# chanchanchan97/ICAFusion

Measured on NVIDIA H100. Metric: 640x512 RGB+IR pairs/sec end-to-end, higher is better.
Workload: dtype f16

## Files before the change

icafusion_b200/csrc/conv_common.cuh:

```cuda
#pragma once
#include "icaf_internal.cuh"

namespace icaf {

constexpr int BM = 128;
constexpr int BK = 64;
constexpr int kLag = 2;
constexpr int kThreads = 288;

enum AMode { A_GATHER = 0, A_TMA2D = 1, A_TMA4D = 2 };

struct ConvProblem {
  const __half* x; const float* bias; const __half* res; __half* y;
  const float* alpha; const float* beta;
  long long x_ld, res_ld, y_ld;
  const float2* ln_stats;
  const float* ln_s;
  float2* stats_out;
};
struct ConvParams {
  ConvProblem p[2];
  int M, N, K, k_pad;
  int B, Hi, Wi, Cin, Ho, Wo, kh, kw, stride, pad;
  int act, epi;
// ... 128 lines not shown
          const float2 r2 = __half22float2(rh[e]);
          rf[2 * e] = r2.x; rf[2 * e + 1] = r2.y;
        }
      } else {
#pragma unroll
        for (int e = 0; e < 8; ++e) rf[e] = 0.f;
      }
      float v[8];
#pragma unroll
      for (int e = 0; e < 8; ++e) v[e] = f(q * 8 + e, rf[e]);
      uint4 o;
      o.x = pack_half2(v[0], v[1]); o.y = pack_half2(v[2], v[3]);
      o.z = pack_half2(v[4], v[5]); o.w = pack_half2(v[6], v[7]);
      if (XM == 2) {
        const __half2* oh = reinterpret_cast<const __half2*>(&o);
#pragma unroll
        for (int e = 0; e < 4; ++e) {
          const float2 w = __half22float2(oh[e]);
          ex.sum += w.x + w.y;
          ex.sumsq += w.x * w.x + w.y * w.y;
        }
      }
      if (do_store) *reinterpret_cast<uint4*>(yp + q * 8) = o;
    }
  } else {
#pragma unroll
    for (int j = 0; j < 32; ++j) {
      if (j < ncols) {
        const float t = f(j, RES != 0 ? __half2float(rp[j]) : 0.f);
        const __half h = __float2half_rn(t);
        if (XM == 2) { const float w = __half2float(h); ex.sum += w; ex.sumsq += w * w; }
        yp[j] = h;
      }
    }
  }
}

__device__ __forceinline__ void load_staged(uint32_t (&acc)[32], const float* p) {
#pragma unroll
  for (int q = 0; q < 8; ++q) {
    const float4 v = *reinterpret_cast<const float4*>(p + 4 * q);
    acc[4 * q] = __float_as_uint(v.x); acc[4 * q + 1] = __float_as_uint(v.y);
    acc[4 * q + 2] = __float_as_uint(v.z); acc[4 * q + 3] = __float_as_uint(v.w);
  }
}

template <bool XM>
__device__ __forceinline__ void epi_dispatch(int mode_act, const uint32_t (&acc)[32], const float* sb, float rbias, float alpha,
                                             float beta, const __half* rp, __half* yp, bool vec, int ncols, EpiRow& ex, int cb) {
  if (XM) {
    switch (mode_act) {
      case 9: epi_chunk<0, 0, 1>(acc, sb, rbias, alpha, beta, rp, yp, vec, ncols, ex, cb); break;
      case 10: epi_chunk<2, 0, 1>(acc, sb, rbias, alpha, beta, rp, yp, vec, ncols, ex, cb); break;
      default: epi_chunk<0, 2, 2>(acc, sb, rbias, alpha, beta, rp, yp, vec, ncols, ex, cb); break;
    }
  } else {
    switch (mode_act) {
      case 0: epi_chunk<0, 0>(acc, sb, rbias, alpha, beta, rp, yp, vec, ncols, ex, cb); break;
      case 1: epi_chunk<0, 1>(acc, sb, rbias, alpha, beta, rp, yp, vec, ncols, ex, cb); break;
      case 2: epi_chunk<0, 2>(acc, sb, rbias, alpha, beta, rp, yp, vec, ncols, ex, cb); break;
      case 3: epi_chunk<1, 0>(acc, sb, rbias, alpha, beta, rp, yp, vec, ncols, ex, cb); break;
      case 4: epi_chunk<1, 1>(acc, sb, rbias, alpha, beta, rp, yp, vec, ncols, ex, cb); break;
      case 5: epi_chunk<1, 2>(acc, sb, rbias, alpha, beta, rp, yp, vec, ncols, ex, cb); break;
      case 6: epi_chunk<2, 0>(acc, sb, rbias, alpha, beta, rp, yp, vec, ncols, ex, cb); break;
      case 7: epi_chunk<2, 1>(acc, sb, rbias, alpha, beta, rp, yp, vec, ncols, ex, cb); break;
      default: epi_chunk<2, 2>(acc, sb, rbias, alpha, beta, rp, yp, vec, ncols, ex, cb); break;
    }
  }
}

template <bool XM>
__device__ __forceinline__ int epi_mode_act(const ConvParams& P, bool has_res) {
  if (XM) return P.ln_parts > 0 ? (P.act == ICAF_ACT_GELU ? 10 : 9) : 11;
  return P.act * 3 + ((P.epi & ICAF_EPI_SCALED_RES) ? 2 : (has_res ? 1 : 0));
}

template <bool XM>
__device__ __forceinline__ void epi_staged_chunk(int mode_act, const uint32_t (&acc)[32], StagedRow& r, const float* sbias,
                                                 float alpha, float beta, int cb, int nb, int N) {
  const int ncols = min(32, N - nb);
  const bool vec = ncols == 32 && ((reinterpret_cast<uintptr_t>(r.yrow + nb) & 15) == 0) &&
                   (!r.rrow || (reinterpret_cast<uintptr_t>(r.rrow + nb) & 15) == 0);
  epi_dispatch<XM>(mode_act, acc, sbias + cb, r.rbias, alpha, beta, r.rrow ? r.rrow + nb : nullptr, r.yrow + nb, vec, ncols,
                   r.ex, cb);
}

constexpr int kOutHalfBytes = BM * 64 * 2;

template <int PP, int NA>
__device__ __forceinline__ void take_cols16(const float (&acc0)[NA], const float (&acc1)[NA], float (&v)[16]) {
  constexpr int Q = PP < NA / 8 ? PP : NA / 8 - 1;
#pragma unroll
  for (int e = 0; e < 8; ++e) { v[e] = acc0[8 * Q + e]; v[8 + e] = acc1[8 * Q + e]; }
}

template <int ACT, int RES>
__device__ __forceinline__ void epi_fragments(const float (&v)[16], uint32_t sa, const float* sb, const float (&rb)[4],
                                              float alpha, float beta) {
#pragma unroll
  for (int h = 0; h < 2; ++h) {
    uint32_t r[4];
    if (RES != 0) ldmatrix_x4(r, sa + 8192u * h);
#pragma unroll
    for (int k = 0; k < 4; ++k) {
      const float2 b = *reinterpret_cast<const float2*>(sb + 8 * (k >> 1));
      const float rbias = rb[2 * h + (k & 1)];
      float2 rf = make_float2(0.f, 0.f);
      if (RES != 0) rf = __half22float2(*reinterpret_cast<const __half2*>(&r[k]));
      r[k] = pack_half2(epi_value<ACT, RES>(v[8 * h + 2 * k], b.x, rbias, rf.x, alpha, beta),
                        epi_value<ACT, RES>(v[8 * h + 2 * k + 1], b.y, rbias, rf.y, alpha, beta));
    }
    stmatrix_x4(sa + 8192u * h, r);
  }
}

__device__ __forceinline__ void epi_fragments_dispatch(int mode_act, const float (&v)[16], uint32_t sa, const float* sb,
                                                       const float (&rb)[4], float alpha, float beta) {
  switch (mode_act) {
    case 0: epi_fragments<0, 0>(v, sa, sb, rb, alpha, beta); break;
    case 1: epi_fragments<0, 1>(v, sa, sb, rb, alpha, beta); break;
    case 2: epi_fragments<0, 2>(v, sa, sb, rb, alpha, beta); break;
    case 3: epi_fragments<1, 0>(v, sa, sb, rb, alpha, beta); break;
    case 4: epi_fragments<1, 1>(v, sa, sb, rb, alpha, beta); break;
    case 5: epi_fragments<1, 2>(v, sa, sb, rb, alpha, beta); break;
    case 6: epi_fragments<2, 0>(v, sa, sb, rb, alpha, beta); break;
    case 7: epi_fragments<2, 1>(v, sa, sb, rb, alpha, beta); break;
    default: epi_fragments<2, 2>(v, sa, sb, rb, alpha, beta); break;
  }
}

template <int NA>
__device__ __forceinline__ void epi_tile_fragments(int mode_act, const float (&acc0)[NA], const float (&acc1)[NA], uint32_t sout,
                                                   const float* sbias, const float (&rb)[4], float alpha, float beta, int w, int l) {
  const uint32_t sa = sout + uint32_t(16 * w + (l & 7) + 8 * ((l >> 3) & 1)) * 128u;
  const float* sb = sbias + 2 * (l & 3);
#pragma unroll 1
  for (int p = 0; p < NA / 8; ++p) {
    float v[16];
    switch (p) {
      case 0: take_cols16<0>(acc0, acc1, v); break;
      case 1: take_cols16<1>(acc0, acc1, v); break;
      case 2: take_cols16<2>(acc0, acc1, v); break;
      case 3: take_cols16<3>(acc0, acc1, v); break;
      case 4: take_cols16<4>(acc0, acc1, v); break;
      case 5: take_cols16<5>(acc0, acc1, v); break;
      case 6: take_cols16<6>(acc0, acc1, v); break;
      default: take_cols16<7>(acc0, acc1, v); break;
    }
    const uint32_t a = sa + uint32_t(p >> 2) * uint32_t(kOutHalfBytes) + (uint32_t((2 * (p & 3) + (l >> 4)) ^ (l & 7)) << 4);
    epi_fragments_dispatch(mode_act, v, a, sb + 16 * p, rb, alpha, beta);
  }
}

__device__ __forceinline__ void fragment_row_bias(float (&rb)[4], const ConvParams& P, const ConvProblem& pr, const TileOrigin& o,
                                                  int w, int l) {
  if ((P.epi & ICAF_EPI_BIAS_ROW) && pr.bias) {
#pragma unroll
    for (int q = 0; q < 4; ++q) {
      int mq;
      bool vq;
      tile_row(P, o, 16 * w + (l >> 2) + 8 * (q & 1) + 64 * (q >> 1), mq, vq);
      rb[q] = vq ? __ldg(pr.bias + mq) : 0.f;
    }
  }
}

template <int BN>
__device__ __forceinline__ void tma_store_tile(const ConvParams& P, const CUtensorMap* map, uint32_t s, int n0, const TileOrigin& o) {
  const int halves = (BN == 128 && n0 + 64 < P.N) ? 2 : 1;
  for (int hh = 0; hh < halves; ++hh) {
    const uint32_t src = s + uint32_t(hh * kOutHalfBytes);
    if (P.a_mode == A_TMA4D) tma_store_4d(map, src, n0 + 64 * hh, o.ox0, o.oy0, o.tb);
    else tma_store_2d(map, src, n0 + 64 * hh, o.m0);
  }
  bulk_commit_group();
}

template <int BN>
__device__ __forceinline__ void tma_load_tile(const ConvParams& P, const CUtensorMap* map, uint32_t s, uint32_t bar, int n0,
                                              const TileOrigin& o) {
  const int halves = (BN == 128 && n0 + 64 < P.N) ? 2 : 1;
  const uint32_t half_bytes = P.a_mode == A_TMA4D ? uint32_t(P.tw * P.th) * 128u : uint32_t(kOutHalfBytes);
  mbar_arrive_expect_tx(bar, uint32_t(halves) * half_bytes);
  for (int hh = 0; hh < halves; ++hh) {
    const uint32_t dst = s + uint32_t(hh * kOutHalfBytes);
    if (P.a_mode == A_TMA4D) tma_load_4d(dst, map, bar, n0 + 64 * hh, o.ox0, o.oy0, o.tb);
    else tma_load_2d(dst, map, bar, n0 + 64 * hh, o.m0);
  }
}

struct ConvPlan {
  int kernel;
  int bn;
  unsigned grid_x, grid_y, grid_z, cluster;
  int smem;
  int tiles, m_tiles, n_tiles;
  int sms;
  bool persist;
  bool stem;
  bool xm;
  int ctas;
};

}
```

icafusion_b200/csrc/conv_gemm.cu:

```cuda
#include <cstdlib>
#include <cstring>

#include "conv_common.cuh"

namespace icaf {

constexpr int kMaxStages = 10;
template <int BN>
struct SmemLayout {
  static constexpr int kABytes = BM * BK * 2;
  static constexpr int kBBytes = BN * BK * 2;
  static constexpr int kStageBytes = kABytes + kBBytes;
  static constexpr int kPitch = BN + 4;
  static constexpr int kAccBytes = BM * kPitch * 4;
  static constexpr int kTailBytes = 256 + BN * 4 + 1024;
  __host__ __device__ static int region(int stages) { return stages * kStageBytes > kAccBytes ? stages * kStageBytes : kAccBytes; }
  static int total(int stages) { return region(stages) + kTailBytes; }
};


template <int BN, bool kTmaA>
__device__ __forceinline__ void load_stage(const ConvParams& P, int a_mode, uint32_t sa, uint32_t bar, uint32_t bytes,
                                           const CUtensorMap* mw, const CUtensorMap* ma, int kb, int n0, const TileOrigin& o) {
  mbar_arrive_expect_tx(bar, bytes);
// ... 379 lines not shown
    mbar_init(order_bar(1), 4);
    mbar_init(res_bar(0), 1);
    mbar_init(res_bar(1), 1);
    for (int h = 0; h < kHaloSlots; ++h) {
      mbar_init(halo_full(h), 1);
      mbar_init(halo_empty(h), 4);
    }
    fence_mbar_init();
  }
  if (tid == 32) {
    tma_prefetch_desc(&maps.w[0]);
    tma_prefetch_desc(&maps.a[0]);
    if (P.tiles > P.m_tiles * P.n_tiles) { tma_prefetch_desc(&maps.w[1]); tma_prefetch_desc(&maps.a[1]); }
    if (!XM) {
      tma_prefetch_desc(&maps.y[0]);
      if (has_res) tma_prefetch_desc(&maps.res[0]);
    }
  }
  __syncthreads();
  pdl_wait();

  if (wg == 0) {
    setmaxnreg_dec<40>();
    if (tid < 32 && elect_one()) {
      const uint32_t a_bytes = a_mode == A_TMA2D ? L::kABytes : uint32_t(P.tw * P.th) * 128u;
      const uint32_t bytes = L::kBBytes + a_bytes;
      int s = 0, h = 0;
      uint32_t ph = 0, hph = 0;
      for (int tile = blockIdx.x; tile < P.tiles; tile += gridDim.x) {
        const PersistTile pt = persist_tile(P, tile);
        const CUtensorMap* mw = pt.z ? &maps.w[1] : &maps.w[0];
        const CUtensorMap* ma = pt.z ? &maps.a[1] : &maps.a[0];
        if (halo) {
          const uint32_t halo_tx = uint32_t((P.tw + 2) * (P.th + 2)) * 128u;
          for (int cb = 0; cb < ncb; ++cb) {
            mbar_wait_quiet(halo_empty(h), hph ^ 1);
            mbar_arrive_expect_tx(halo_full(h), halo_tx);
            tma_load_4d(smem_base + uint32_t(kStages * PL::kFilterBytes + h * P.halo_bytes), ma, halo_full(h), cb * BK,
                        pt.o.ox0 - 1, pt.o.oy0 - 1, pt.o.tb);
            if (++h == kHaloSlots) { h = 0; hph ^= 1; }
            for (int tap = 0; tap < 9; ++tap) {
              mbar_wait_quiet(empty_bar(s), ph ^ 1);
              mbar_arrive_expect_tx(full_bar(s), PL::kFilterBytes);
              tma_load_2d(smem_base + uint32_t(s * PL::kFilterBytes), mw, full_bar(s), tap * P.Cin + cb * BK, pt.n0);
              if (++s == kStages) { s = 0; ph ^= 1; }
            }
          }
          continue;
        }
        for (int kb = 0; kb < nkb; ++kb) {
          mbar_wait_quiet(empty_bar(s), ph ^ 1);
          load_stage<128, true>(P, a_mode, smem_base + s * L::kStageBytes, full_bar(s), bytes, mw, ma, kb, pt.n0, pt.o);
          if (++s == kStages) { s = 0; ph ^= 1; }
        }
      }
    }
    return;
  }

  setmaxnreg_inc<232>();
  const int c = wg - 1;
  const int t = tid & 127, w = t >> 5, l = t & 31;
  const int bar_id = 2 + c;
  const uint32_t sout = smem_base + ring_bytes + uint32_t(c * PL::kOutBytes);
  float* sacc = reinterpret_cast<float*>(smem_gen + ring_bytes + c * PL::kOutBytes);
  float* sbias = reinterpret_cast<float*>(smem_gen + bar_off + 256 + c * 128 * 4);
  int lane_px[2];
#pragma unroll
  for (int hm = 0; hm < 2; ++hm) {
    int m = 64 * hm + 16 * w + (l & 7) + 8 * ((l >> 3) & 1);
    if (m > P.tw * P.th - 1) m = P.tw * P.th - 1;
    const int py = P.tw ? m / P.tw : 0;
    lane_px[hm] = py * (P.tw + 2) + m - py * P.tw;
  }
  for (int tile = blockIdx.x + c * gridDim.x; tile < P.tiles; tile += 2 * gridDim.x) {
    const int j = (tile - int(blockIdx.x)) / int(gridDim.x);
    const PersistTile pt = persist_tile(P, tile);
    const ConvProblem pr = pick_problem(P, pt.z);
    const int n0 = pt.n0;
    const TileOrigin& o = pt.o;
    const float bias_r = (pr.bias && !(P.epi & ICAF_EPI_BIAS_ROW) && n0 + t < P.N) ? __ldg(pr.bias + n0 + t) : 0.f;
    float alpha = 0.f, beta = 1.f;
    if (P.epi & ICAF_EPI_SCALED_RES) { alpha = __ldg(pr.alpha); beta = __ldg(pr.beta); }
    StagedRow sr;
    float rb[4] = {0.f, 0.f, 0.f, 0.f};
    if (XM) {
      staged_row<128, XM>(sr, P, pr, o, t, n0);
    } else {
      fragment_row_bias(rb, P, pr, o, w, l);
      if (t == 0) {
        bulk_wait_group_read<0>();
        if (has_res) tma_load_tile<128>(P, pt.z ? &maps.res[1] : &maps.res[0], sout, res_bar(c), n0, o);
      }
      sbias[t] = bias_r;
      named_bar_sync(bar_id, 128);
    }

    float acc0[64], acc1[64];
#pragma unroll
    for (int i = 0; i < 64; ++i) { acc0[i] = 0.f; acc1[i] = 0.f; }
    auto hand_back = [&](int s) { if (l == 0) mbar_arrive(empty_bar(s)); };
    auto halo_back = [&](int h) { if (l == 0) mbar_arrive(halo_empty(h)); };
    const int g0 = j * nkb;
    if (j > 0) mbar_wait_quiet(order_bar(c), uint32_t((j >> 1) - (1 - c)) & 1u);
    int s_last, h_last = 0;
    if (halo) {
      halo_mma_loop(acc0, acc1, P, smem_base, kStages, g0, j * ncb, lane_px, l, full_bar, halo_full, hand_back, halo_back,
                    s_last, h_last);
    } else {
      s_last = mma_loop<128>(acc0, acc1, smem_base, kStages, nkb, g0 % kStages, uint32_t(g0 / kStages) & 1u, full_bar,
                             hand_back);
    }
    if (l == 0) mbar_arrive(order_bar(c ^ 1));
    wgmma_wait<0>();
    hand_back(s_last);
    if (halo) halo_back(h_last);

    if constexpr (!XM) {
      if (has_res) mbar_wait_quiet(res_bar(c), uint32_t(j >> 1) & 1u);
      epi_tile_fragments<64>(epi_mode_act<false>(P, has_res), acc0, acc1, sout, sbias, rb, alpha, beta, w, l);
      fence_proxy_async_smem();
      named_bar_sync(bar_id, 128);
      if (t == 0) {
        tma_store_tile<128>(P, pt.z ? &maps.y[1] : &maps.y[0], sout, n0, o);
        if (tile + 2 * int(gridDim.x) >= P.tiles) bulk_wait_group<0>();
      }
      continue;
    }

    const int mode_act = epi_mode_act<XM>(P, has_res);
    const float* arow = sacc + size_t(t) * PL::kPitch;
#pragma unroll 1
    for (int cc = 0; cc < 4; ++cc) {
      named_bar_sync(bar_id, 128);
      if (cc == 0) sbias[t] = bias_r;
      switch (cc) {
        case 0: stage_chunk<0>(acc0, acc1, sacc, w, l); break;
        case 1: stage_chunk<1>(acc0, acc1, sacc, w, l); break;
        case 2: stage_chunk<2>(acc0, acc1, sacc, w, l); break;
        default: stage_chunk<3>(acc0, acc1, sacc, w, l); break;
      }
      named_bar_sync(bar_id, 128);
      const int cb = 32 * cc;
      if (sr.mvalid && n0 + cb < P.N) {
        uint32_t acc[32];
        load_staged(acc, arow);
        epi_staged_chunk<XM>(mode_act, acc, sr, sbias, alpha, beta, cb, n0 + cb, P.N);
      }
    }
    if (mode_act == 11 && sr.mvalid && n0 < P.N) epi_row_emit(sr.ex, P, pr, sr.m, n0, min(n0 + 128, P.N));
  }
}

constexpr int kStemThreads = 128;
struct StemLayout {
  static constexpr int kFilterBytes = 3 * SmemLayout<64>::kBBytes;
  static constexpr int kBiasOff = kFilterBytes;
  static constexpr int kBarOff = kBiasOff + 64 * 4;
  static constexpr int kHaloOff = kFilterBytes + 1024;
  __host__ __device__ static int pitch(int Wo) { return (Wo < BM ? Wo : BM) + 2; }
  __host__ __device__ static int runs(int Wo) { return 1 + (BM - 1 + Wo - 1) / Wo; }
  static int total(int Wo) {
    const int halo = runs(Wo) * 3 * pitch(Wo) * 32;
    return kHaloOff + (halo > kOutHalfBytes ? halo : kOutHalfBytes) + 1024;
  }
};

__global__ void __launch_bounds__(kStemThreads, 4)
conv_stem_kernel(const ConvParams P, const __grid_constant__ ConvMaps maps) {
  extern __shared__ uint8_t smem_raw[];
  using SL = StemLayout;
  const uint32_t smem_base = (smem_u32(smem_raw) + 1023u) & ~1023u;
  uint8_t* smem_gen = smem_raw + (smem_base - smem_u32(smem_raw));
  const uint32_t bar = smem_base + SL::kBarOff;
  const uint32_t halo = smem_base + SL::kHaloOff;
  float* sbias = reinterpret_cast<float*>(smem_gen + SL::kBiasOff);

  pdl_launch_dependents();
  const int t = threadIdx.x, w = t >> 5, l = t & 31;
  const int bz = blockIdx.z, n0 = blockIdx.y * 64;
  const ConvProblem pr = pick_problem(P, bz);
  const TileOrigin o{int(blockIdx.x) * BM, 0, 0, 0};
  const int g0 = o.m0 / P.Wo, ox0 = o.m0 - g0 * P.Wo;
  const int len0 = min(P.Wo - ox0, BM);
  const int nruns = 1 + (BM - len0 + P.Wo - 1) / P.Wo;
  const int pitch = SL::pitch(P.Wo);
  int lane_hp[2];
#pragma unroll
  for (int hm = 0; hm < 2; ++hm) {
    const int r = 64 * hm + 16 * w + (l & 7) + 8 * ((l >> 3) & 1);
    int j = 0, p = r;
    if (r >= len0) {
      const int q = (r - len0) / P.Wo;
      j = 1 + q;
      p = r - len0 - q * P.Wo;
    }
    lane_hp[hm] = 3 * j * pitch + p;
  }
  if (t == 0) {
    mbar_init(bar, 1);
    fence_mbar_init();
  }
  if (t == 32) {
    tma_prefetch_desc(bz ? &maps.w[1] : &maps.w[0]);
    tma_prefetch_desc(bz ? &maps.y[1] : &maps.y[0]);
  }
  __syncthreads();
  pdl_wait();

  if (t == 0) {
    const CUtensorMap* mw = bz ? &maps.w[1] : &maps.w[0];
    mbar_arrive_expect_tx(bar, SL::kFilterBytes);
#pragma unroll 1
    for (int kb = 0; kb < 3; ++kb) tma_load_2d(smem_base + uint32_t(kb * SmemLayout<64>::kBBytes), mw, bar, kb * BK, n0);
  }
  if (t < 64) sbias[t] = (pr.bias && !(P.epi & ICAF_EPI_BIAS_ROW) && n0 + t < P.N) ? __ldg(pr.bias + n0 + t) : 0.f;
  float rb[4] = {0.f, 0.f, 0.f, 0.f};
  fragment_row_bias(rb, P, pr, o, w, l);

  const int c = t & 1;
#pragma unroll 1
  for (int j = 0; j < nruns; ++j) {
    const int g = g0 + j;
    const int xs = j ? 0 : ox0;
    const int len = j ? min(P.Wo, BM - len0 - (j - 1) * P.Wo) : len0;
    const int b = g / P.Ho, oy = g - b * P.Ho;
    const bool gv = g < P.B * P.Ho;
#pragma unroll
    for (int ty = 0; ty < 3; ++ty) {
      const int iy = oy + ty - 1;
      const bool rv = gv && (unsigned)iy < (unsigned)P.Hi;
      const __half* src = pr.x + (rv ? (size_t(b) * P.Hi + iy) * P.Wi * pr.x_ld : 0) + 8 * c;
      const int h0 = (3 * j + ty) * pitch;
      for (int px = t >> 1; px < len + 2; px += kStemThreads / 2) {
        const int ix = xs - 1 + px, h = h0 + px;
        const bool ok = rv && (unsigned)ix < (unsigned)P.Wi;
        cp_async16(halo + uint32_t(h) * 32u + (uint32_t(c ^ ((h >> 2) & 1)) << 4), ok ? src + size_t(ix) * pr.x_ld : pr.x, ok);
      }
    }
  }
  cp_async_commit();
  cp_async_wait<0>();
  __syncthreads();
  mbar_wait_quiet(bar, 0);

  float acc0[32], acc1[32];
#pragma unroll
  for (int i = 0; i < 32; ++i) { acc0[i] = 0.f; acc1[i] = 0.f; }
  uint32_t fa[3][2][4];
#pragma unroll
  for (int tap = 0; tap < 9; ++tap) {
    const int f = tap % 3;
    const int off = (tap / 3) * pitch + tap % 3;
#pragma unroll
    for (int hm = 0; hm < 2; ++hm) {
      const int h = lane_hp[hm] + off;
      ldmatrix_x4(fa[f][hm], halo + uint32_t(h) * 32u + (uint32_t((l >> 4) ^ ((h >> 2) & 1)) << 4));
    }
    wgmma_fence();
    const uint64_t bd = gmma_desc_sw128(smem_base + uint32_t((tap >> 2) * SmemLayout<64>::kBBytes + 32 * (tap & 3)));
    wgmma_rs<0>(acc0, fa[f][0], bd, tap != 0);
    wgmma_rs<0>(acc1, fa[f][1], bd, tap != 0);
    wgmma_commit();
    wgmma_wait<2>();
  }
  wgmma_wait<0>();
  __syncthreads();

  epi_tile_fragments<32>(epi_mode_act<false>(P, false), acc0, acc1, halo, sbias, rb, 0.f, 1.f, w, l);
  fence_proxy_async_smem();
  __syncthreads();
  if (t == 0) {
    tma_store_tile<64>(P, bz ? &maps.y[1] : &maps.y[0], halo, n0, o);
    bulk_wait_group<0>();
  }
}

struct SimtParams { ConvParams P; const __half* w[2]; };
__global__ void conv_gemm_simt_kernel(const SimtParams S) {
  pdl_launch_dependents();
  pdl_wait();
  const ConvParams& P = S.P;
  const ConvProblem pr = pick_problem(P, blockIdx.z);
  const __half* w = blockIdx.z ? S.w[1] : S.w[0];
  long long idx = blockIdx.x * (long long)blockDim.x + threadIdx.x;
  if (idx >= (long long)P.M * P.N) return;
  int n = int(idx % P.N);
  int m = int(idx / P.N);
  int ox = m % P.Wo, t = m / P.Wo, oy = t % P.Ho, b = t / P.Ho;
  float acc = 0.f;
  for (int ky = 0; ky < P.kh; ++ky)
    for (int kx = 0; kx < P.kw; ++kx) {
      int iy = oy * P.stride - P.pad + ky, ix = ox * P.stride - P.pad + kx;
      if ((unsigned)iy >= (unsigned)P.Hi || (unsigned)ix >= (unsigned)P.Wi) continue;
      const __half* xp = pr.x + (size_t(b) * P.Hi * P.Wi + size_t(iy) * P.Wi + ix) * pr.x_ld;
      const __half* wp = w + size_t(n) * P.k_pad + (ky * P.kw + kx) * P.Cin;
      for (int c = 0; c < P.Cin; ++c) acc += __half2float(xp[c]) * __half2float(wp[c]);
    }
  if (pr.bias) acc += (P.epi & ICAF_EPI_BIAS_ROW) ? pr.bias[m] : pr.bias[n];
  if (P.act == ICAF_ACT_SILU) acc = acc / (1.0f + expf(-acc));
  else if (P.act == ICAF_ACT_GELU) acc = gelu_erf_f(acc);
  if (pr.res) {
    float rf = __half2float(pr.res[size_t(m) * pr.res_ld + n]);
    acc = (P.epi & ICAF_EPI_SCALED_RES) ? (*pr.alpha) * rf + (*pr.beta) * acc : acc + rf;
  }
  pr.y[size_t(m) * pr.y_ld + n] = __float2half_rn(acc);
}

static int fill_geom(const icaf_conv_geom* g, int n_io, ConvParams& P) {
  if (!g || n_io < 1 || n_io > 2) return set_error(ICAF_ERR_BAD_ARG, "conv2d: need 1 or 2 problems");
  if (!(g->Cin == 4 || g->Cin % 8 == 0)) return set_error(ICAF_ERR_UNSUPPORTED, "conv2d: Cin must be 4 or a multiple of 8");
  if (g->Cin == 4 && (g->Wi % 2 || g->stride % 2 || g->pad % 2 || g->kw % 2))
    return set_error(ICAF_ERR_UNSUPPORTED, "conv2d: packed-image (Cin=4) path needs even Wi, stride, pad, kw");
  if (g->k_pad % 64 || g->k_pad < g->kh * g->kw * g->Cin) return set_error(ICAF_ERR_BAD_ARG, "conv2d: bad k_pad");
  if (g->w_rows < g->Cout) return set_error(ICAF_ERR_BAD_ARG, "conv2d: w_rows < Cout");
  long long M = (long long)g->B * g->Ho * g->Wo;
  if (M <= 0 || M > 0x7fffffffLL || (long long)g->B * g->Hi * g->Wi > 0x7fffffffLL)
    return set_error(ICAF_ERR_BAD_ARG, "conv2d: size out of range");
  if ((g->epi & (ICAF_EPI_ADD_RES | ICAF_EPI_SCALED_RES)) == (ICAF_EPI_ADD_RES | ICAF_EPI_SCALED_RES))
    return set_error(ICAF_ERR_BAD_ARG, "conv2d: ADD_RES and SCALED_RES are exclusive");
  if ((g->epi & ICAF_EPI_LN_FOLD) && ((g->epi & ~ICAF_EPI_LN_FOLD) != 0 || !(g->act == ICAF_ACT_NONE || g->act == ICAF_ACT_GELU) ||
                                      g->kh != 1 || g->kw != 1 || g->stride != 1 || g->pad != 0))
    return set_error(ICAF_ERR_UNSUPPORTED, "conv2d: LN_FOLD is a linear-layer (1x1) epilogue without residual, activation none / GELU");
  if ((g->epi & ICAF_EPI_EMIT_STATS) && ((g->epi & ~ICAF_EPI_EMIT_STATS) != ICAF_EPI_SCALED_RES || g->act != ICAF_ACT_NONE))
    return set_error(ICAF_ERR_UNSUPPORTED, "conv2d: EMIT_STATS rides on the SCALED_RES epilogue without activation");
  P.M = int(M); P.N = g->Cout; P.K = g->kh * g->kw * g->Cin; P.k_pad = g->k_pad;
  P.B = g->B; P.Hi = g->Hi; P.Wi = g->Wi; P.Cin = g->Cin; P.Ho = g->Ho; P.Wo = g->Wo;
  P.kh = g->kh; P.kw = g->kw; P.stride = g->stride; P.pad = g->pad; P.act = g->act; P.epi = g->epi;
  P.a_mode = A_GATHER; P.tw = P.th = P.tiles_x = P.tiles_y = 0; P.stages = 2; P.splits = 1; P.cblk = 64;
  P.ln_parts = 0; P.ln_eps = 0.f; P.ln_inv_k = 0.f;
  P.m_tiles = P.n_tiles = P.tiles = 0;
  P.tma_epi = 0;
  P.halo_bytes = 0;
  memset(P.p, 0, sizeof(P.p));
  return ICAF_OK;
}

static int fill_params(const icaf_conv_geom* g, const icaf_conv_io* io, int n_io, ConvParams& P, const __half* (&w)[2]) {
  if (!io) return set_error(ICAF_ERR_BAD_ARG, "conv2d: null io");
  if (int rc = fill_geom(g, n_io, P)) return rc;
  for (int i = 0; i < 2; ++i) {
    const icaf_conv_io& s = io[i < n_io ? i : 0];
    bool need_res = g->epi & (ICAF_EPI_ADD_RES | ICAF_EPI_SCALED_RES);
    if (!s.x || !s.w || !s.y || (need_res && !s.res) || ((g->epi & ICAF_EPI_SCALED_RES) && (!s.alpha || !s.beta)))
      return set_error(ICAF_ERR_BAD_ARG, "conv2d: null pointer");
    if ((reinterpret_cast<uintptr_t>(s.x) & 15) || (reinterpret_cast<uintptr_t>(s.w) & 15) || (s.x_ld % 8 && g->Cin != 4) ||
        (g->Cin == 4 && s.x_ld != 4))
      return set_error(ICAF_ERR_BAD_ARG, "conv2d: x / w must be 16-byte aligned with x_ld a multiple of 8");
    if ((g->epi & ICAF_EPI_LN_FOLD) && (!s.ln_stats || !s.ln_colsum || s.ln_parts < 1 || s.ln_parts > 64))
      return set_error(ICAF_ERR_BAD_ARG, "conv2d: LN_FOLD needs ln_stats, ln_colsum and 1..64 partials per row");
    if ((g->epi & ICAF_EPI_EMIT_STATS) && !s.stats_out) return set_error(ICAF_ERR_BAD_ARG, "conv2d: EMIT_STATS needs stats_out");
    if (i > 0 && (g->epi & ICAF_EPI_LN_FOLD) && (s.ln_parts != io[0].ln_parts || s.ln_eps != io[0].ln_eps))
      return set_error(ICAF_ERR_BAD_ARG, "conv2d: grouped problems must share ln_parts / ln_eps");
    P.p[i] = ConvProblem{(const __half*)s.x, s.bias, need_res ? (const __half*)s.res : nullptr, (__half*)s.y, s.alpha, s.beta,
                         s.x_ld, s.res_ld, s.y_ld,
                         (g->epi & ICAF_EPI_LN_FOLD) ? (const float2*)s.ln_stats : nullptr,
                         (g->epi & ICAF_EPI_LN_FOLD) ? s.ln_colsum : nullptr,
                         (g->epi & ICAF_EPI_EMIT_STATS) ? (float2*)s.stats_out : nullptr};
    if (i == 0 && (g->epi & ICAF_EPI_LN_FOLD)) { P.ln_parts = s.ln_parts; P.ln_eps = s.ln_eps; P.ln_inv_k = 1.0f / float(P.K); }
    w[i] = (const __half*)s.w;
  }
  return ICAF_OK;
}

static void plan_a_mode(const icaf_conv_geom* g, ConvParams& P) {
  if (g->kh == 1 && g->kw == 1 && g->stride == 1 && g->pad == 0 && g->Cin % 8 == 0) {
    P.a_mode = A_TMA2D;
    return;
  }
  if (g->Cin % 64 == 0 && g->stride <= 2) {
    int best_tw = 0, best_th = 0;
    double best_u = 0.0;
    for (int tw = 1; tw <= 128 && tw <= g->Wo; ++tw) {
      if (g->Wo % tw || tw * g->stride > 256) continue;
      int th = 128 / tw;
      if (th > g->Ho) th = g->Ho;
      if (th * g->stride > 256) th = 256 / g->stride;
      int ty = (g->Ho + th - 1) / th;
      double u = double(g->Wo) * g->Ho / (double(g->Wo / tw) * ty * 128.0);
      if (u > best_u + 1e-9 || (u > best_u - 1e-9 && tw > best_tw)) { best_u = u; best_tw = tw; best_th = th; }
    }
    if (best_u >= 0.6) {
      P.a_mode = A_TMA4D; P.tw = best_tw; P.th = best_th; P.tiles_x = g->Wo / best_tw; P.tiles_y = (g->Ho + best_th - 1) / best_th;
    }
  }
}

template <int BN>
static int plan_tc(ConvParams& P, int n_io, ConvPlan& pl) {
  using L = SmemLayout<BN>;
  constexpr int kSmemCap = 227 * 1024;
  const int mt = P.a_mode == A_TMA4D ? P.B * P.tiles_x * P.tiles_y : (P.M + BM - 1) / BM;
  if (P.a_mode == A_TMA4D && !(P.tw >= 1 && P.th >= 1 && P.tw * P.th <= BM && P.tiles_x * P.tw >= P.Wo && P.tiles_y * P.th >= P.Ho &&
                               P.cblk == 64 && P.Cin % 64 == 0))
    return set_error(ICAF_ERR_BAD_ARG, "conv2d(tc): 4-D tiles must cover the map with at most 128 pixels each, 64-channel blocks");
  unsigned gx = unsigned(mt), gy = unsigned((P.N + BN - 1) / BN), gz = unsigned(n_io);
  const long long tiles = (long long)gx * gy * gz;
  const int budget = (tiles <= pl.sms || BN > 64) ? kSmemCap : (kSmemCap / 2 - 1024);
  int stages = (budget - L::kTailBytes) / L::kStageBytes;
  const int nkb = P.k_pad / BK;
  if (stages > nkb) stages = nkb;
  if (stages > kMaxStages) stages = kMaxStages;
  if (stages < 2) stages = 2;
  int splits = 1;
  if (tiles * 2 <= pl.sms && nkb >= 8) {
    splits = int(pl.sms / tiles);
    if (splits > 8) splits = 8;
    if (splits > nkb / 4) splits = nkb / 4;
    if (splits < 1) splits = 1;
  }
  if (splits > 1) {
    const int per = (nkb + splits - 1) / splits;
    if (stages > per) stages = per < 2 ? 2 : per;
    gx *= splits;
  }
  if (stages > kMaxStages || L::total(stages) > kSmemCap)
    return set_error(ICAF_ERR_BAD_ARG, "conv2d(tc): shared-memory plan exceeds the ring / 227 KB");
  P.stages = stages;
  P.splits = splits;
  pl.kernel = ICAF_KERNEL_TC; pl.bn = BN;
  pl.grid_x = gx; pl.grid_y = gy; pl.grid_z = gz; pl.cluster = unsigned(splits);
  pl.smem = L::total(stages);
  pl.tiles = int(tiles); pl.m_tiles = mt; pl.n_tiles = int(gy);
  pl.persist = false; pl.ctas = int(gx * gy * gz);
  return ICAF_OK;
}

static int plan_persist(ConvParams& P, ConvPlan& pl) {
  constexpr int kSmemCap = 227 * 1024;
  const bool halo = !pl.xm && P.a_mode == A_TMA4D && P.kh == 3 && P.kw == 3 && P.stride == 1 && P.pad == 1;
  P.halo_bytes = halo ? ((P.tw + 2) * (P.th + 2) * 128 + 1023) / 1024 * 1024 : 0;
  int stages = kMaxStages;
  while (stages > 2 && PersistLayout::total(stages, P.halo_bytes) > kSmemCap) --stages;
  if (PersistLayout::total(stages, P.halo_bytes) > kSmemCap)
    return set_error(ICAF_ERR_BAD_ARG, "conv2d(persist): shared-memory plan exceeds 227 KB");
  P.stages = stages;
  P.m_tiles = pl.m_tiles; P.n_tiles = pl.n_tiles; P.tiles = pl.tiles;
  pl.persist = true;
  pl.ctas = pl.tiles < pl.sms ? pl.tiles : pl.sms;
  pl.smem = PersistLayout::total(stages, P.halo_bytes);
  return ICAF_OK;
}

template <int BN>
static int encode_maps(const ConvParams& P, const __half* const (&w)[2], const icaf_conv_geom* g, int n_io, bool out_maps,
                       ConvMaps& maps) {
  memset(&maps, 0, sizeof(maps));
  for (int i = 0; i < n_io; ++i) {
    int rc = encode_tmap_2d(&maps.w[i], w[i], (uint64_t)P.k_pad, (uint64_t)g->w_rows, (uint64_t)P.k_pad * 2, BK, BN);
    if (rc) return rc;
    const ConvProblem& pr = P.p[i];
    if (P.a_mode == A_TMA2D)
      rc = encode_tmap_2d(&maps.a[i], pr.x, (uint64_t)P.Cin, (uint64_t)P.M, (uint64_t)pr.x_ld * 2, BK, BM);
    else if (P.a_mode == A_TMA4D && P.halo_bytes)
      rc = encode_tmap_nhwc(&maps.a[i], pr.x, P.Cin, P.Wi, P.Hi, P.B, pr.x_ld, BK, P.tw + 2, P.th + 2, 1, 1);
    else if (P.a_mode == A_TMA4D)
      rc = encode_tmap_nhwc(&maps.a[i], pr.x, P.Cin, P.Wi, P.Hi, P.B, pr.x_ld, BK, P.tw * P.stride, P.th * P.stride, P.stride,
                            P.stride);
    if (rc) return rc;
    if (out_maps) {
      auto out_map = [&](CUtensorMap* m, const __half* base, long long ld) {
        return P.a_mode != A_TMA4D ? encode_tmap_2d(m, base, (uint64_t)P.N, (uint64_t)P.M, (uint64_t)ld * 2, 64, BM)
                                   : encode_tmap_nhwc(m, base, P.N, P.Wo, P.Ho, P.B, ld, 64, P.tw, P.th, 1, 1);
      };
      if ((rc = out_map(&maps.y[i], pr.y, pr.y_ld))) return rc;
      if (pr.res && (rc = out_map(&maps.res[i], pr.res, pr.res_ld))) return rc;
    }
  }
  if (n_io == 1) { maps.w[1] = maps.w[0]; maps.a[1] = maps.a[0]; maps.y[1] = maps.y[0]; maps.res[1] = maps.res[0]; }
  return ICAF_OK;
}

template <int BN>
static int launch_conv(const ConvParams& P, const ConvPlan& pl, const __half* const (&w)[2], const icaf_conv_geom* g, int n_io,
                       cudaStream_t st) {
  void (*kernel)(ConvParams, ConvMaps) = pl.xm ? conv_gemm_tc_kernel<BN, true> : conv_gemm_tc_kernel<BN, false>;
  if (pl.persist) kernel = pl.xm ? conv_gemm_persist_kernel<true> : conv_gemm_persist_kernel<false>;
  if (pl.stem) kernel = conv_stem_kernel;
  static bool configured[3][2][kMaxDevices] = {};
  const int family = pl.stem ? 2 : (pl.persist ? 1 : 0);
  if (int rc = configure_smem(kernel, 227 * 1024, configured[family][pl.xm], "conv2d: cudaFuncSetAttribute")) return rc;
  ConvMaps maps;
  if (int rc = encode_maps<BN>(P, w, g, n_io, P.tma_epi != 0, maps)) return rc;
  const dim3 grid = pl.persist ? dim3(unsigned(pl.ctas)) : dim3(pl.grid_x, pl.grid_y, pl.grid_z);
  const int threads = pl.persist ? kPersistThreads : (pl.stem ? kStemThreads : kThreads);
  return launch_kc("conv2d_fwd", kernel, grid, dim3(threads), (size_t)pl.smem, st, pl.cluster, P, maps);
}

static int plan_conv(const icaf_conv_geom* g, int n_io, int sms, bool tma_out, ConvParams& P, ConvPlan& pl) {
  memset(&pl, 0, sizeof(pl));
  pl.sms = sms;
  if (sms < 1) return set_error(ICAF_ERR_BAD_ARG, "conv2d: SM count must be positive");
  pl.xm = (P.epi & (ICAF_EPI_LN_FOLD | ICAF_EPI_EMIT_STATS)) != 0;
  plan_a_mode(g, P);
  const long long mt = P.a_mode == A_TMA4D ? (long long)P.B * P.tiles_x * P.tiles_y : (P.M + BM - 1) / BM;
  auto ctas = [&](int bn) { return mt * ((P.N + bn - 1) / bn) * n_io; };
  int bn = 32;
  if (P.N > 64 && ctas(128) >= sms) bn = 128;
  else if (P.N > 32 && ctas(64) >= sms) bn = 64;
  int rc;
  switch (bn) {
    case 128:
      rc = plan_tc<128>(P, n_io, pl);
      if (!rc && (pl.xm || tma_out) && P.a_mode != A_GATHER && P.splits == 1 && pl.tiles > sms) rc = plan_persist(P, pl);
      break;
    case 64:
      rc = plan_tc<64>(P, n_io, pl);
      if (!rc && !pl.xm && tma_out && P.a_mode == A_GATHER && P.splits == 1 && P.Cin == 16 && P.kh == 3 && P.kw == 3 &&
          P.stride == 1 && P.pad == 1 && !(P.epi & (ICAF_EPI_ADD_RES | ICAF_EPI_SCALED_RES))) {
        P.stages = 1;
        pl.stem = true;
        pl.smem = StemLayout::total(P.Wo);
      }
      break;
    default: rc = plan_tc<32>(P, n_io, pl); break;
  }
  if (rc) return rc;
  P.tma_epi = !pl.xm && (pl.persist || (tma_out && P.splits == 1 && pl.bn >= 64)) ? 1 : 0;
  return ICAF_OK;
}

}

using namespace icaf;


extern "C" int icaf_conv2d_plan(const icaf_conv_geom* g, int n_io, int sm_count, int pair_mode, icaf_conv_plan* out) {
  if (!out) return set_error(ICAF_ERR_BAD_ARG, "conv2d_plan: null output");
  ConvParams P;
  int rc = fill_geom(g, n_io, P);
  if (rc) return rc;
  ConvPlan pl;
  (void)pair_mode;
  rc = plan_conv(g, n_io, sm_count, true, P, pl);
  if (rc) return rc;
  out->kernel = pl.kernel; out->bn = pl.bn; out->a_mode = P.a_mode;
  out->tile_w = P.tw; out->tile_h = P.th; out->tiles_x = P.tiles_x; out->tiles_y = P.tiles_y;
  out->cblk = P.cblk; out->halo = 0; out->stages = P.stages; out->splits = P.splits;
  out->grid_x = int(pl.grid_x); out->grid_y = int(pl.grid_y); out->grid_z = int(pl.grid_z); out->cluster = int(pl.cluster);
  out->smem_bytes = pl.smem; out->work_items = pl.tiles; out->ctas = pl.ctas;
  return ICAF_OK;
}

extern "C" int icaf_conv2d_fwd(const icaf_conv_geom* g, const icaf_conv_io* io, int n_io, void* stream) {
  ConvParams P;
  const __half* w[2];
  int rc = fill_params(g, io, n_io, P, w);
  if (rc) return rc;
  bool tma_out = true;
  for (int i = 0; i < n_io; ++i) {
    const ConvProblem& pr = P.p[i];
    tma_out = tma_out && (reinterpret_cast<uintptr_t>(pr.y) & 15) == 0 && pr.y_ld % 8 == 0 &&
              (!pr.res || ((reinterpret_cast<uintptr_t>(pr.res) & 15) == 0 && pr.res_ld % 8 == 0));
  }
  ConvPlan pl;
  rc = plan_conv(g, n_io, sm_count_cached(), tma_out, P, pl);
  if (rc) return rc;
  cudaStream_t st = (cudaStream_t)stream;
  switch (pl.bn) {
    case 128: return launch_conv<128>(P, pl, w, g, n_io, st);
    case 64: return launch_conv<64>(P, pl, w, g, n_io, st);
    case 32: return launch_conv<32>(P, pl, w, g, n_io, st);
    default: return set_error(ICAF_ERR_BAD_ARG, "conv2d: the planner produced an unknown tile width");
  }
}

extern "C" int icaf_conv2d_fwd_simt(const icaf_conv_geom* g, const icaf_conv_io* io, int n_io, void* stream) {
  SimtParams S;
  int rc = fill_params(g, io, n_io, S.P, S.w);
  if (rc) return rc;
  long long total = (long long)S.P.M * S.P.N;
  dim3 grid(blocks_for(total, 256), 1, n_io);
  return launch_k("conv2d_fwd_simt", conv_gemm_simt_kernel, dim3(grid), dim3(256), 0, (cudaStream_t)stream, S);
}
```

Before: 2196.

## Add persistent streaming kernel for small-K pointwise convs with resident filter slice

Adds a warp-specialized persistent kernel for 1x1 (TMA2D) convolutions with K up to 256. It loads the CTA's whole filter slice into shared memory once, then streams only activation tiles through a ring. Two consumer warpgroup pairs alternate M-tiles, ordered by barriers, and each runs its epilogue with stmatrix and TMA stores. The aim is to stop reloading filter tiles per K-block and to overlap one pair's epilogue with the other's MMA. The cost is extra planning complexity and a 640-thread register rebalance.

```diff
diff --git a/icafusion_b200/csrc/conv_common.cuh b/icafusion_b200/csrc/conv_common.cuh
--- a/icafusion_b200/csrc/conv_common.cuh
+++ b/icafusion_b200/csrc/conv_common.cuh
@@ -304,6 +304,31 @@
   }
 }
 
+template <int ACT>
+__device__ __forceinline__ void epi_block_fragments(const float (&acc)[64], uint32_t sout, const float* sbias, const float (&rb)[4],
+                                                    int w, int l) {
+  const uint32_t sa = sout + uint32_t(16 * w + (l & 7) + 8 * ((l >> 3) & 1)) * 128u;
+#pragma unroll
+  for (int hh = 0; hh < 2; ++hh) {
+    uint32_t r[16];
+#pragma unroll
+    for (int q = 0; q < 4; ++q) {
+      const int p = 4 * hh + q;
+#pragma unroll
+      for (int k = 0; k < 4; ++k) {
+        const float2 b = *reinterpret_cast<const float2*>(sbias + 16 * p + 8 * (k >> 1) + 2 * (l & 3));
+        r[4 * q + k] = pack_half2(epi_value<ACT, 0>(acc[8 * p + 2 * k], b.x, rb[k & 1], 0.f, 0.f, 1.f),
+                                  epi_value<ACT, 0>(acc[8 * p + 2 * k + 1], b.y, rb[k & 1], 0.f, 0.f, 1.f));
+      }
+    }
+#pragma unroll
+    for (int q = 0; q < 4; ++q) {
+      const uint32_t a = sa + uint32_t(hh * kOutHalfBytes) + (uint32_t((2 * q + (l >> 4)) ^ (l & 7)) << 4);
+      stmatrix_x4(a, *reinterpret_cast<const uint32_t(*)[4]>(&r[4 * q]));
+    }
+  }
+}
+
 __device__ __forceinline__ void fragment_row_bias(float (&rb)[4], const ConvParams& P, const ConvProblem& pr, const TileOrigin& o,
                                                   int w, int l) {
   if ((P.epi & ICAF_EPI_BIAS_ROW) && pr.bias) {
@@ -350,6 +375,7 @@
   int sms;
   bool persist;
   bool stem;
+  bool stream;
   bool xm;
   int ctas;
 };
diff --git a/icafusion_b200/csrc/conv_gemm.cu b/icafusion_b200/csrc/conv_gemm.cu
--- a/icafusion_b200/csrc/conv_gemm.cu
+++ b/icafusion_b200/csrc/conv_gemm.cu
@@ -555,6 +555,142 @@
   }
 }
 
+constexpr int kStreamThreads = 640;
+constexpr int kStreamRegsLaunch = (65536 / kStreamThreads) & ~7, kStreamRegsLow = 24, kStreamRegsHigh = 112;
+static_assert(128 * kStreamRegsLow + 512 * kStreamRegsHigh <= kStreamThreads * kStreamRegsLaunch,
+              "register rebalance exceeds the launch allocation");
+struct StreamLayout {
+  static constexpr int kABytes = SmemLayout<128>::kABytes;
+  static constexpr int kFilterBoxBytes = SmemLayout<128>::kBBytes;
+  static constexpr int kOutBytes = 2 * kOutHalfBytes;
+  __host__ __device__ static int ring_off(int nkb) { return nkb * kFilterBoxBytes; }
+  __host__ __device__ static int out_off(int nkb, int stages) { return ring_off(nkb) + stages * kABytes; }
+  __host__ __device__ static int bar_off(int nkb, int stages) { return out_off(nkb, stages) + 2 * kOutBytes; }
+  static int total(int nkb, int stages) { return bar_off(nkb, stages) + 256 + 128 * 4 + 1024; }
+};
+
+__global__ void __launch_bounds__(kStreamThreads, 1)
+pointwise_stream_kernel(const ConvParams P, const __grid_constant__ ConvMaps maps) {
+  extern __shared__ uint8_t smem_raw[];
+  using SL = StreamLayout;
+  const uint32_t smem_base = (smem_u32(smem_raw) + 1023u) & ~1023u;
+  uint8_t* smem_gen = smem_raw + (smem_base - smem_u32(smem_raw));
+  const int kStages = P.stages;
+  const int nkb = P.k_pad / BK;
+  const uint32_t ring = smem_base + uint32_t(SL::ring_off(nkb));
+  const uint32_t bar_base = smem_base + uint32_t(SL::bar_off(nkb, kStages));
+  auto full_bar = [&](int s) { return bar_base + 8u * s; };
+  auto empty_bar = [&](int s) { return bar_base + 8u * (kMaxStages + s); };
+  auto order_bar = [&](int p) { return bar_base + 8u * (2 * kMaxStages + p); };
+  const uint32_t filter_bar = bar_base + 8u * (2 * kMaxStages + 2);
+  float* sbias = reinterpret_cast<float*>(smem_gen + SL::bar_off(nkb, kStages) + 256);
+
+  pdl_launch_dependents();
+  const int tid = threadIdx.x;
+  const int nslices = P.tiles / P.m_tiles;
+  const int slice = int(blockIdx.x) % nslices;
+  const int ctas_s = int(gridDim.x) / nslices + (slice < int(gridDim.x) % nslices ? 1 : 0);
+  const int mt0 = int(blockIdx.x) / nslices;
+  const int z = slice / P.n_tiles;
+  const int n0 = (slice - z * P.n_tiles) * 128;
+  if (tid == 0) {
+    for (int s = 0; s < kStages; ++s) {
+      mbar_init(full_bar(s), 1);
+      mbar_init(empty_bar(s), 8);
+    }
+    mbar_init(order_bar(0), 8);
+    mbar_init(order_bar(1), 8);
+    mbar_init(filter_bar, 1);
+    fence_mbar_init();
+  }
+  if (tid == 512) {
+    tma_prefetch_desc(z ? &maps.w[1] : &maps.w[0]);
+    tma_prefetch_desc(z ? &maps.a[1] : &maps.a[0]);
+    tma_prefetch_desc(z ? &maps.y[1] : &maps.y[0]);
+  }
+  __syncthreads();
+  pdl_wait();
+
+  if (tid >= 512) {
+    setmaxnreg_dec<kStreamRegsLow>();
+    if (tid < 544 && elect_one()) {
+      const CUtensorMap* mw = z ? &maps.w[1] : &maps.w[0];
+      const CUtensorMap* ma = z ? &maps.a[1] : &maps.a[0];
+      mbar_arrive_expect_tx(filter_bar, uint32_t(nkb * SL::kFilterBoxBytes));
+      for (int kb = 0; kb < nkb; ++kb) tma_load_2d(smem_base + uint32_t(kb * SL::kFilterBoxBytes), mw, filter_bar, kb * BK, n0);
+      int s = 0;
+      uint32_t ph = 0;
+      for (int mt = mt0; mt < P.m_tiles; mt += ctas_s) {
+        for (int kb = 0; kb < nkb; ++kb) {
+          mbar_wait_quiet(empty_bar(s), ph ^ 1);
+          mbar_arrive_expect_tx(full_bar(s), SL::kABytes);
+          tma_load_2d(ring + uint32_t(s * SL::kABytes), ma, full_bar(s), kb * BK, mt * BM);
+          if (++s == kStages) { s = 0; ph ^= 1; }
+        }
+      }
+    }
+    return;
+  }
+
+  setmaxnreg_inc<kStreamRegsHigh>();
+  const int wg = tid >> 7, pair = wg >> 1, h = wg & 1;
+  const int t = tid & 127, w = t >> 5, l = t & 31;
+  const int pt = tid & 255;
+  const int bar_id = 1 + pair;
+  const uint32_t sout = smem_base + uint32_t(SL::out_off(nkb, kStages) + pair * SL::kOutBytes);
+  const ConvProblem pr = pick_problem(P, z);
+  const CUtensorMap* my = z ? &maps.y[1] : &maps.y[0];
+  if (tid < 128) sbias[tid] = (pr.bias && !(P.epi & ICAF_EPI_BIAS_ROW) && n0 + tid < P.N) ? __ldg(pr.bias + n0 + tid) : 0.f;
+  named_bar_sync(3, 512);
+  mbar_wait_quiet(filter_bar, 0);
+  auto hand_back = [&](int s) { if (l == 0) mbar_arrive(empty_bar(s)); };
+
+  for (int j = pair;; j += 2) {
+    const int mt = mt0 + j * ctas_s;
+    if (mt >= P.m_tiles) break;
+    if (pt == 0) bulk_wait_group_read<0>();
+    named_bar_sync(bar_id, 256);
+
+    float acc[64];
+#pragma unroll
+    for (int i = 0; i < 64; ++i) acc[i] = 0.f;
+    const int g0 = j * nkb;
+    if (j > 0) mbar_wait_quiet(order_bar(pair), uint32_t((j >> 1) - (1 - pair)) & 1u);
+    int s = g0 % kStages, s_prev = s;
+    uint32_t ph = uint32_t(g0 / kStages) & 1u;
+    for (int kb = 0; kb < nkb; ++kb) {
+      mbar_wait_quiet(full_bar(s), ph);
+      const uint32_t sa = ring + uint32_t(s * SL::kABytes) + uint32_t(h * 64 * 128);
+      const uint32_t sb = smem_base + uint32_t(kb * SL::kFilterBoxBytes);
+      wgmma_fence();
+#pragma unroll
+      for (int k = 0; k < BK / 16; ++k) wgmma_ss<0, 0>(acc, gmma_desc_sw128(sa + 32 * k), gmma_desc_sw128(sb + 32 * k), (kb | k) != 0);
+      wgmma_commit();
+      wgmma_wait<1>();
+      if (kb > 0) hand_back(s_prev);
+      s_prev = s;
+      if (++s == kStages) { s = 0; ph ^= 1; }
+    }
+    if (l == 0) mbar_arrive(order_bar(pair ^ 1));
+    wgmma_wait<0>();
+    hand_back(s_prev);
+
+    const TileOrigin o{mt * BM, 0, 0, 0};
+    float rb[4] = {0.f, 0.f, 0.f, 0.f};
+    fragment_row_bias(rb, P, pr, TileOrigin{o.m0 + 64 * h, 0, 0, 0}, w, l);
+    const uint32_t sblock = sout + uint32_t(h * 64 * 128);
+    if (P.act == ICAF_ACT_SILU) epi_block_fragments<ICAF_ACT_SILU>(acc, sblock, sbias, rb, w, l);
+    else if (P.act == ICAF_ACT_GELU) epi_block_fragments<ICAF_ACT_GELU>(acc, sblock, sbias, rb, w, l);
+    else epi_block_fragments<ICAF_ACT_NONE>(acc, sblock, sbias, rb, w, l);
+    fence_proxy_async_smem();
+    named_bar_sync(bar_id, 256);
+    if (pt == 0) {
+      tma_store_tile<128>(P, my, sout, n0, o);
+      if (mt + 2 * ctas_s >= P.m_tiles) bulk_wait_group<0>();
+    }
+  }
+}
+
 constexpr int kStemThreads = 128;
 struct StemLayout {
   static constexpr int kFilterBytes = 3 * SmemLayout<64>::kBBytes;
@@ -845,6 +981,20 @@
   return ICAF_OK;
 }
 
+static bool plan_stream(ConvParams& P, ConvPlan& pl) {
+  constexpr int kSmemCap = 227 * 1024;
+  const int nkb = P.k_pad / BK;
+  if (!pl.persist || pl.xm || P.a_mode != A_TMA2D || P.k_pad > 256 || (P.epi & (ICAF_EPI_ADD_RES | ICAF_EPI_SCALED_RES)) ||
+      pl.tiles / pl.m_tiles > pl.ctas)
+    return false;
+  int stages = kMaxStages;
+  while (stages > 2 && StreamLayout::total(nkb, stages) > kSmemCap) --stages;
+  P.stages = stages;
+  pl.stream = true;
+  pl.smem = StreamLayout::total(nkb, stages);
+  return true;
+}
+
 template <int BN>
 static int encode_maps(const ConvParams& P, const __half* const (&w)[2], const icaf_conv_geom* g, int n_io, bool out_maps,
                        ConvMaps& maps) {
@@ -879,14 +1029,15 @@
                        cudaStream_t st) {
   void (*kernel)(ConvParams, ConvMaps) = pl.xm ? conv_gemm_tc_kernel<BN, true> : conv_gemm_tc_kernel<BN, false>;
   if (pl.persist) kernel = pl.xm ? conv_gemm_persist_kernel<true> : conv_gemm_persist_kernel<false>;
+  if (pl.stream) kernel = pointwise_stream_kernel;
   if (pl.stem) kernel = conv_stem_kernel;
-  static bool configured[3][2][kMaxDevices] = {};
-  const int family = pl.stem ? 2 : (pl.persist ? 1 : 0);
+  static bool configured[4][2][kMaxDevices] = {};
+  const int family = pl.stream ? 3 : (pl.stem ? 2 : (pl.persist ? 1 : 0));
   if (int rc = configure_smem(kernel, 227 * 1024, configured[family][pl.xm], "conv2d: cudaFuncSetAttribute")) return rc;
   ConvMaps maps;
   if (int rc = encode_maps<BN>(P, w, g, n_io, P.tma_epi != 0, maps)) return rc;
   const dim3 grid = pl.persist ? dim3(unsigned(pl.ctas)) : dim3(pl.grid_x, pl.grid_y, pl.grid_z);
-  const int threads = pl.persist ? kPersistThreads : (pl.stem ? kStemThreads : kThreads);
+  const int threads = pl.stream ? kStreamThreads : (pl.persist ? kPersistThreads : (pl.stem ? kStemThreads : kThreads));
   return launch_kc("conv2d_fwd", kernel, grid, dim3(threads), (size_t)pl.smem, st, pl.cluster, P, maps);
 }
 
@@ -906,6 +1057,7 @@
     case 128:
       rc = plan_tc<128>(P, n_io, pl);
       if (!rc && (pl.xm || tma_out) && P.a_mode != A_GATHER && P.splits == 1 && pl.tiles > sms) rc = plan_persist(P, pl);
+      if (!rc) plan_stream(P, pl);
       break;
     case 64:
       rc = plan_tc<64>(P, n_io, pl);
```

After: 2249, median of 6. 1.02x the previous value.
